# Nemesis1303/gFedNTM

Measured on AMD Instinct MI355X. Metric: docs/sec (whole node) + NPMI, ProdLDA K=50 8-client fed on synthetic BoW, higher is better.
Workload: dtype fp32

## Files before the change

### csrc/gfk_common.h

```cpp
#pragma once

#include <hip/hip_runtime.h>
#include <stdint.h>

#define GFK_MAX_LAYERS 8
#define GFK_MAX_SEGS 48
#define GFK_ADAM_CHUNK 256
#define GFK_WAVE 64

extern "C" {

enum GfkAct { GFK_SOFTPLUS = 0, GFK_RELU = 1, GFK_SIGMOID = 2, GFK_TANH = 3,
              GFK_LEAKYRELU = 4, GFK_ELU = 5, GFK_SELU = 6, GFK_RRELU = 7 };

enum GfkModelKind { GFK_PRODLDA = 0, GFK_LDA = 1 };

enum GfkInput { GFK_IN_BOW = 0, GFK_IN_COMBINED = 1, GFK_IN_CONTEXTUAL = 2 };

typedef struct GfkModel {
  int32_t bmax;
  int32_t V, K;
  int32_t n_hidden;
  int32_t H[GFK_MAX_LAYERS];
  int32_t act;
// ... 80 lines not shown
  int32_t ctx_kb, ctx_ckb;
  int32_t slot_cap;
  int32_t* ws_sidx;
  float* ws_sval;
  int32_t mm_bf16;
  int32_t ctx_parts;

  int32_t lab_on;
  int32_t lab_off;
  const float* labels;
  float *w_cls, *b_cls;
  float *ws_lab;
  float *ws_dlab;
  float *ws_ce;
  float *ws_thd;
  int32_t lab_in_enc;
  int32_t bwd_pre;
  float* ws_dt;
  const void* dev;
  const void* dev_upd;
  int32_t n_batch;
  int32_t ldb;
  int32_t ctx_bgrid;
  float* ws_colstat;
  float* kl_hist;
  float* rl_hist;
  int64_t off_own;
} GfkModel;

constexpr int GFK_FWD_POSTFOLD = 65536;
constexpr int GFK_LB = 524288;
constexpr int GFK_POST_ROWS2 = 1048576;
constexpr int GFK_POST_JOINT = 2097152;
constexpr int GFK_POST_ROWS4 = 4194304;
constexpr int GFK_BWD_BATCH8 = 8388608;
__host__ __device__ __forceinline__ int gfk_post_joint_rows(int stage_flags) {
  return !(stage_flags & GFK_POST_JOINT) ? 1 : (stage_flags & GFK_POST_ROWS4) ? 4 : 2;
}
constexpr int GFK_BMAX_LIMIT = 512;
__host__ __device__ __forceinline__ int gfk_hlast(const GfkModel& m) {
  int h = m.H[0];
#pragma unroll
  for (int l = 1; l < GFK_MAX_LAYERS; ++l) {
#if defined(__HIP_DEVICE_COMPILE__)
    const int hl = __builtin_amdgcn_readfirstlane(m.H[l]);
#else
    const int hl = m.H[l];
#endif
    if (l < m.n_hidden) h = hl;
  }
// ... 564 lines not shown
```

### csrc/posterior.hip

```cpp
#define GFK_BATCHED_COPY 1
#include "gfk_common.h"
#include "gfk_launch.h"

using namespace gfk;

namespace {
constexpr int PT = 256;
constexpr int FT = 1024;
__host__ __device__ inline int pad4(int x) { return (x + 3) & ~3; }

__device__ __forceinline__ float quad_sum(float v) {
  v += dpp_f<0xB1>(v);
  return v + dpp_f<0x4E>(v);
}

__host__ __device__ inline int post_hmax(const GfkModel& m) {
  int h = 0;
#pragma unroll
  for (int l = 0; l < GFK_MAX_LAYERS; ++l)
    if (l < m.n_hidden) h = h > m.H[l] ? h : m.H[l];
  return h;
}

__host__ __device__ inline int post_weight_floats(const GfkModel& m) {
// ... 361 lines not shown
  if (m.lab_on) post_label_head(m, red, row, nb, tid);
  GFK_STAMP(m, 3);
}

extern "C" size_t gfk_row_bwd_smem(const GfkModel* m) { return sizeof(float) * 4 * (size_t)pad4(m->K); }

__device__ __forceinline__ void post_term_hist(const GfkModel& m, int nb, int step0, float* scratch,
                                               int tid, int nt) {
  float k = 0.f, r = 0.f;
  for (int b = tid; b < nb; b += nt) {
    k += m.ws_kl[b];
    r += m.ws_rl[b];
  }
  lds_barrier();
  const float ks = block_sum_wave0(k, scratch);
  lds_barrier();
  const float rs = block_sum_wave0(r, scratch);
  if (tid == 0) {
    m.kl_hist[step0] = ks / (float)nb;
    m.rl_hist[step0] = rs / (float)nb;
  }
}

__device__ __forceinline__ void post_batch_level(const GfkModel& m, int nb, float* scratch, int tid) {
  __shared__ float red[3 * PT];
  const int K = m.K;
  const float wk = m.kl_weight;
  const int step0 = *m.step;
  float lterm = 0.f;
  for (int b = tid; b < nb; b += PT)
    lterm += wk * m.ws_kl[b] + m.ws_rl[b] + (m.lab_on ? m.ws_ce[b] : 0.f);
  if (m.learn_priors) {
    constexpr int RB = 16;
    const int cw = K <= 64 ? 64 : K <= 128 ? 128 : PT, ng = PT / cw;
    const int c = tid % cw, g = tid / cw;
    for (int k0 = 0; k0 < K; k0 += cw) {
      const int k = k0 + c, kk = min(k, K - 1);
      const float pm = m.prior_mean[kk];
      float smu = 0.f, svar = 0.f, sdm2 = 0.f;
      for (int r0 = g; r0 < nb; r0 += RB * ng) {
        float mu[RB], ls[RB];
#pragma unroll
        for (int i = 0; i < RB; ++i) {
          const int r = min(r0 + ng * i, nb - 1);
          mu[i] = m.ws_mu[r * K + kk];
          ls[i] = m.ws_ls[r * K + kk];
        }
#pragma unroll
        for (int i = 0; i < RB; ++i)
          if (r0 + ng * i < nb) {
            smu += mu[i];
            svar += expf(ls[i]);
            const float dm = pm - mu[i];
            sdm2 += dm * dm;
          }
      }
      red[tid] = smu;
      red[PT + tid] = svar;
      red[2 * PT + tid] = sdm2;
      lds_barrier();
      if (g == 0 && k < K) {
        for (int j = 1; j < ng; ++j) {
          smu += red[c + j * cw];
          svar += red[PT + c + j * cw];
          sdm2 += red[2 * PT + c + j * cw];
        }
        const float pv = m.prior_var[k];
        m.prior_mean[k + m.off_g] = wk * ((float)nb * pm - smu) / pv;
        m.prior_var[k + m.off_g] = wk * 0.5f * ((float)nb / pv - svar / (pv * pv) - sdm2 / (pv * pv));
      }
      lds_barrier();
    }
  }
  const float l = block_sum_wave0(lterm, scratch);
  if (tid == 0) {
    m.loss_hist[step0] = l;
    *m.step = step0 + 1;
  }
  if (m.kl_hist) post_term_hist(m, nb, step0, scratch, tid, PT);
}

template <int KQ, bool GB = false>
__global__ void __launch_bounds__(PT) gfk_row_bwd_k(GfkArgT<GB> ga) {
  const GfkModel& m = gfk_model(ga);
  extern __shared__ __attribute__((aligned(16))) float part[];
  int K = m.K, B = m.bmax, np = m.n_dpart + (m.lab_on ? 1 : 0);
  const float* dpart = m.ws_dthetad;
  const int32_t* nbp = m.ws_nb;
  keep(K, B, np, dpart, nbp);
  const int tid = threadIdx.x, lane = tid & 63, wave = uniform(tid >> 6);
  const int row = gfk_bx();
  const int nb = *nbp;
  if ((m.stage_flags & GFK_POST_ROWS2) && row == B) {
    post_batch_level(m, nb, part, tid);
    return;
  }
  if (row >= nb) return;
  GFK_STAMP(m, 8);
  constexpr int U = 32 / KQ;
// ... 288 lines not shown
  for (int q = 0; q < CQ; ++q) rs[q] = m.ws_bn_rstd[min(tid + q * FT, 2 * K - 1)];
  float lterm = 0.f, pmk = 0.f, pvk = 1.f;
  int step0 = 0;
  if (extra) {
    if (tid < nb) lterm = m.kl_weight * m.ws_kl[tid] + m.ws_rl[tid] + (m.lab_on ? m.ws_ce[tid] : 0.f);
    if (tid < K) { pmk = m.prior_mean[tid]; pvk = m.prior_var[tid]; }
    if (tid == 0) step0 = *m.step;
  }
  if (row >= nb && !extra) {
    vm_barrier();
    return;
  }
  vm_barrier();
  GFK_STAMP(m, 11);

  const float* dmu = in_lds ? smem + L.dmu : dmu_g;
  const float* dls = in_lds ? smem + L.dls : dls_g;
  const float* mu = in_lds ? smem + L.mu : mu_g;
  const float* ls = in_lds ? smem + L.ls : ls_g;
  float* S = smem + L.sums;
  const int P2 = pad4(2 * K);
  const float inv_nb = 1.f / (float)nb;
  if (extra) {
    const float* pmean = smem + L.pm;
    if constexpr (in_lds) {
      for (int cb = 0; cb < 2 * K; cb += FT / 16) {
        const int c2 = cb + (tid >> 4), g = tid & 15;
        const bool valid = c2 < 2 * K;
        const int k = c2 < K ? c2 : c2 - K;
        const float* xh = c2 < K ? mu : ls;
        const float pm = pmean[k];
        float s3 = 0.f, s4 = 0.f;
        if (valid)
#pragma unroll 4
          for (int r = g; r < nb; r += 16) {
            const float x = xh[r * LD + k];
            s3 += c2 < K ? x : expf(x);
            const float dm = pm - x;
            s4 += c2 < K ? dm * dm : 0.f;
          }
        s3 = row16_sum(s3);
        s4 = row16_sum(s4);
        if (valid && g == 0) {
          S[2 * P2 + c2] = s3;
          S[3 * P2 + c2] = s4;
        }
      }
    } else if constexpr (PS) {
      for (int c = tid; c < 2 * K; c += FT) {
        S[2 * P2 + c] = m.ws_colstat[8 * K + c];
        S[3 * P2 + c] = m.ws_colstat[10 * K + c];
      }
    } else {
      if (B <= 64) post_prior_sums<32>(K, nb, mu, ls, pmean, S + 2 * P2, S + 3 * P2, smem + L.red2, tid);
      else post_prior_sums<64>(K, nb, mu, ls, pmean, S + 2 * P2, S + 3 * P2, smem + L.red2, tid);
    }
    lds_barrier();
    const float wk = m.kl_weight;
    if (tid < K && m.learn_priors) {
      const float sdm2 = S[3 * P2 + tid];
      const float smu = S[2 * P2 + tid], svar = S[2 * P2 + K + tid];
      m.prior_mean[tid + m.off_g] = wk * ((float)nb * pmk - smu) / pvk;
      m.prior_var[tid + m.off_g] =
          wk * 0.5f * ((float)nb / pvk - svar / (pvk * pvk) - sdm2 / (pvk * pvk));
    }
    const float l = block_sum_wave0(lterm, smem + L.red);
    if (tid == 0) {
      m.loss_hist[step0] = l;
      *m.step = step0 + 1;
    }
    if (m.kl_hist) post_term_hist(m, nb, step0, smem + L.red, tid, FT);
    return;
  }
  if constexpr (in_lds) {
    for (int cb = 0; cb < 2 * K; cb += FT / 16) {
      const int c2 = cb + (tid >> 4), g = tid & 15;
      const bool valid = c2 < 2 * K;
      const int k = c2 < K ? c2 : c2 - K;
      const float* dy = c2 < K ? dmu : dls;
      const float* xh = c2 < K ? mu : ls;
      float s1 = 0.f, s2 = 0.f;
      if (valid)
#pragma unroll 4
        for (int r = g; r < nb; r += 16) {
          const float d = dy[r * LD + k], x = xh[r * LD + k];
          s1 += d;
          s2 += d * x;
        }
      s1 = row16_sum(s1);
      s2 = row16_sum(s2);
      if (valid && g == 0) {
// ... 398 lines not shown
```

### gfedntm_amd/data/bow.py

```python
from __future__ import annotations

import dataclasses
from typing import Dict, List, Optional, Sequence

import numpy as np
import scipy.sparse as sp
import torch
from torch.utils.data import Dataset


def to_csr(x) -> sp.csr_matrix:
    if isinstance(x, torch.Tensor):
        x = x.detach().cpu().numpy()
    m = sp.csr_matrix(x, dtype=np.float32)
    m.sum_duplicates()
    m.sort_indices()
    return m


class BOWDataset(Dataset):

    def __init__(self, X, idx2token):
        self.csr = to_csr(X)
        self.idx2token = idx2token
# ... 117 lines not shown
    def n_steps(self) -> int:
        return len(self.start)

    @staticmethod
    def build(n_docs: int, batch_size: int, n_steps: int, seed: int = 0) -> "BatchPlan":
        if n_docs <= 0:
            raise ValueError("empty shard")
        per_epoch = -(-n_docs // batch_size)
        n_epochs = -(-n_steps // per_epoch) if n_steps else 0
        rng = np.random.default_rng(seed)
        order = np.concatenate([rng.permutation(n_docs) for _ in range(max(n_epochs, 1))])
        s = np.arange(n_steps)
        ep, mb = s // per_epoch, s % per_epoch
        start = ep * n_docs + mb * batch_size
        size = np.minimum(batch_size, n_docs - mb * batch_size)
        return BatchPlan(order.astype(np.int32), start.astype(np.int32), size.astype(np.int32),
                         ep.astype(np.int32), mb.astype(np.int32), mb == per_epoch - 1,
                         n_docs, batch_size)

    def batch(self, step: int) -> np.ndarray:
        return self.order[self.start[step]: self.start[step] + self.size[step]]


def corpus_from_texts(texts: Sequence[str], vocabulary: Dict[str, int]) -> sp.csr_matrix:
    from .vocab import vectorize
    return vectorize(texts, vocabulary)


def stack_shards(shards: List[sp.csr_matrix]) -> sp.csr_matrix:
    return sp.vstack(shards, format="csr")
```

### gfedntm_amd/federation/client.py

```python
from __future__ import annotations

import datetime
import logging
from typing import List, Optional

import numpy as np
import torch

from ..data.bow import BatchPlan
from ..eval.export import postprocess_thetas, save_model_as_npz


class FederatedClient:
    def __init__(self, client_id: int, tm, dataset, max_iters: int, logger=None, seed: int = 0,
                 save_path: Optional[str] = None, log_every: int = 0, n_samples: int = 20,
                 epoch_snapshots: bool = False, agg: str = "params"):
        if agg not in ("params", "grads"):
            raise ValueError("agg must be 'params' (FedAvg) or 'grads' (gradient all-reduce)")
        self.agg = agg
        self.id = client_id
        self.tm = tm
        self.dataset = dataset
        self.logger = logger or logging.getLogger(f"gfedntm_amd.client{client_id}")
        self.save_path = save_path
        self.log_every = log_every
        self.n_samples = n_samples
        self.epoch_snapshots = epoch_snapshots
        tm.train_data = dataset
        self.data = tm.device_data(dataset)
        self.n_docs = self.data.n_docs
        self.max_iters = max_iters
        self.plan = BatchPlan.build(self.n_docs, tm.batch_size, max_iters, seed=seed)
        if agg == "grads" and tm.backend == "fused":
            from ..ops.engine import UPDATE_GRAD
            tm.engine.set_update_mode(UPDATE_GRAD)
        tm.engine.bind_data(self.data, self.plan)
        if hasattr(tm.engine, "own_rng"):
            tm.engine.own_rng(seed)
        tm.model.train()
        self.weight: Optional[float] = None
        self.ground_truth = None
        self.synthetic_eval: Optional[dict] = None
        self.current_mb = 0
        self.current_epoch = 0
        self.samples_processed = 0
        self.train_loss = 0.0
        self.epoch_first_step = 0
        self.results_saved = False
        tm.best_components = tm.model.beta
        self._pending: List[tuple] = []
        self._pinned = None
        self._events: List = []
        self._slot = 0
        hist = tm.engine.loss_hist
        if hist.device.type == "cuda":
            self._pinned = torch.zeros(64, dtype=torch.float32, pin_memory=True)
            self._events = [torch.cuda.Event() for _ in range(self._pinned.numel())]
            self._pinned[:1].copy_(hist[:1].sum().view(1), non_blocking=True)
            torch.cuda.synchronize(hist.device)

    @property
    def shared(self) -> torch.Tensor:
        return self.tm.flat.shared

    @property
    def fused(self) -> bool:
        return self.tm.backend == "fused"

    def set_fedavg_weight(self, w: float):
        self.weight = float(w)
        if self.fused and self.agg == "params":
            self.tm.engine.set_fedavg_scale(self.weight)

    def enable_graph(self, on: bool = True):
        if self.fused:
            self.tm.engine.enable_graph(on)

    def local_step(self, it: int):
        if self.agg == "grads":
            self.tm.engine.compute_grads(it)
            if self.weight is not None:
                self.shared_grads.mul_(self.weight)
            return
        self.tm.engine.step(it)
        if self.weight is not None and not self.fused:
# ... 34 lines not shown
                                 self.current_mb, loss, self.samples_processed,
                                 float(e.kl_hist[it].item()), float(e.rl_hist[it].item()))
            else:
                self.logger.info("-- -- Minibatch %d loss %s / samples processes %d", self.current_mb,
                                 loss, self.samples_processed)
        self.current_mb += 1
        if bool(self.plan.epoch_end[it]):
            self._queue_epoch_summary(self.epoch_first_step, it)
            if self.epoch_snapshots and self.save_path:
                self.flush()
                self.save_results(self.save_path.replace(".npz", f"_epoch_{self.current_epoch}.npz"))
            self.current_epoch += 1
            self.current_mb = 0
            self.epoch_first_step = it + 1
        if self.current_epoch >= self.tm.num_epochs and not self.results_saved:
            self.flush()
            self.logger.info("Epoch end reached")
            if self.save_path:
                self.save_results(self.save_path)
            self.results_saved = True
        self.poll()
        return self.results_saved

    def _queue_epoch_summary(self, first: int, last: int):
        hist = self.tm.engine.loss_hist
        if hist.device.type != "cuda":
            self._pending.append((self.current_epoch, self.samples_processed,
                                  float(hist[first: last + 1].sum()), None))
            self.poll()
            return
        if len(self._pending) >= self._pinned.numel():
            self.flush()
        slot = self._slot
        self._slot = (slot + 1) % self._pinned.numel()
        dst = self._pinned[slot: slot + 1]
        dst.copy_(hist[first: last + 1].sum().view(1), non_blocking=True)
        ev = self._events[slot]
        ev.record()
        self._pending.append((self.current_epoch, self.samples_processed, dst, ev))

    def _emit(self, epoch: int, samples: int, epoch_loss: float):
        self.train_loss += epoch_loss
        self.train_loss /= samples
        self.logger.info("Epoch: [%d/%d]\tSamples: [%d/%d]\tTrain Loss: %s\tTime: %s",
                         epoch + 1, self.tm.num_epochs, samples,
                         self.n_docs * self.tm.num_epochs, self.train_loss,
                         datetime.datetime.now())
# ... 71 lines not shown
```

### gfedntm_amd/federation/rank_round.py

```python
from __future__ import annotations

import os
from typing import Dict, List, Optional

import torch

from ..parallel.aggregator import (LOCAL_ALL, LOCAL_BCAST, LOCAL_FIRST, LOCAL_REFRESH,
                                   LOCAL_SHARED, LOCAL_SHARED_ALL, CollectiveAggregator,
                                   local_fedavg, prepare_local_fedavg)
from ..utils.misc import graph_capture
from .client import FederatedClient


def inplace_threshold_bytes() -> int:
    return int(float(os.environ.get("GFEDNTM_XGMI_INPLACE_MB", "8")) * (1 << 20))


class SingleClientRound:

    def __init__(self, client: FederatedClient, world: int, device, on_gpu_plane: bool,
                 allreduce: Optional[str], agg_mode: str, bucket_bytes: int, logger,
                 wire: str = "fp32"):
        self.clients = [client]
        self.client = client
        self.agg_mode = agg_mode
        if wire != "fp32" and agg_mode != "params":
            raise ValueError("fedavg_wire bf16delta averages parameters (agg_mode 'params')")
        self.wire = wire
        self.agg = CollectiveAggregator(bucket_bytes=bucket_bytes, method="rccl", wire=wire,
                                        weight=client.weight if wire != "fp32" else None)
        self.agg.set_reference(client.shared)
        self.in_step = None
        if on_gpu_plane and client.fused and agg_mode == "params" and world > 1:
            self.in_step = client.tm.engine.attach_fedavg(method=allreduce, wire=wire)
            logger.info("-- -- FedAvg all-reduce: %s", self.in_step)
        self.method = self.in_step if self.in_step else (None if world == 1 else "rccl")
        self.attach = getattr(client.tm.engine, "fedavg_attach", None) if self.in_step else None

    @property
    def xgmi(self) -> bool:
        return bool(self.in_step) and self.in_step.startswith("xgmi")

    def rounds_per_replay(self) -> int:
        c = self.client
        if not (c.fused and self.agg_mode == "params" and c.tm.engine.steps_per_replay_ok()
                and (self.in_step is not None or self.agg.world == 1)):
            return 1
        return max(1, int(os.environ.get("GFEDNTM_ROUNDS_PER_GRAPH", "16")))

    def prewarm(self, kmax: int):
        e = self.client.tm.engine
        if self.rounds_per_replay() <= 1 or e.plan is None:
            return
        e.warm_graph()
        k = 2
        while k <= kmax:
            if k not in e._graphs_k:
                e._capture(k)
            k *= 2

# ... 20 lines not shown
            self.agg.allreduce_(c.shared)

    def resync_reference(self):
        if self.wire == "fp32":
            return
        self.agg.set_reference(self.client.shared)
        if self.in_step is not None:
            self.client.tm.engine.fedavg_set_reference()

    def error(self) -> int:
        e = self.client.tm.engine
        return e.fedavg_error() if self.in_step is not None and self.client.fused else 0

    def error_async(self):
        self.client.tm.engine.fedavg_error_async()

    def error_poll(self) -> int:
        return self.client.tm.engine.fedavg_error_poll()

    def debug(self) -> dict:
        return self.client.tm.engine.fedavg_debug() if self.in_step is not None else {}

    def close(self):
        if self.in_step is not None and self.client.fused:
            self.client.tm.engine.detach_fedavg()
            self.in_step = None


class MultiClientRound:

    def __init__(self, clients: List[FederatedClient], world: int, device, on_gpu_plane: bool,
                 allreduce: Optional[str], graph: bool, logger, wire: str = "fp32"):
        self.clients = clients
        self.wire = wire
        self.weight = sum(c.weight for c in clients) if wire != "fp32" else None
        self.device = device
        self.world = world
        self.shared = [c.shared for c in clients]
        engines = [c.tm.engine for c in clients]
        self.fused = all(c.fused for c in clients) and device.type == "cuda"
        n = self.shared[0].numel()
        self.parts: Dict[str, tuple] = {"rest": (0, n)}
        from ..ops.engine import UPDATE_FUSED
        if (self.fused and world > 1 and on_gpu_plane
                and all(e.update_mode == UPDATE_FUSED for e in engines)):
            self.parts = dict(engines[0].fedavg_parts())
# ... 11 lines not shown
                           "inplace": {k: c.xgmi is not None and c.xgmi.data is not None
                                       for k, c in self.colls.items()},
                           "tuning": {k: c.tuning for k, c in self.colls.items() if c.tuning},
                           "plane": {k: c.describe() for k, c in self.colls.items()}}
        self.coll_in_graph = bool(self.colls) and all(c.xgmi is not None for c in self.colls.values())
        if not self.coll_in_graph and len(self.parts) > 1:
            for c in self.colls.values():
                if c.xgmi is not None:
                    c.xgmi.close()
                    c.xgmi = None
            self.parts = {"rest": (0, n)}
            coll = CollectiveAggregator(method="rccl", wire=wire, weight=self.weight)
            coll.prepare(self.shared[0])
            self.colls = {"rest": coll}
        self.method = (None if world == 1 else
                       "xgmi" + ("+overlap" if len(self.parts) > 1 else "")
                       if self.coll_in_graph else self.colls["rest"].active)
        self.graph = (graph and self.fused and not any(e.host_gemm_fallback for e in engines))
        if self.graph:
            for c in clients:
                c.enable_graph(False)
        if self.fused:
            prepare_local_fedavg(self.shared)
        self.fold_plan: Optional[str] = None
        self._g = None
        self._gk: Dict[int, object] = {}
        self._gm: Dict[int, object] = {}
        self._bss: Dict[tuple, object] = {}
        self._shared_plan: Optional[bool] = None
        self._shared_why: Optional[str] = None
        self._S: Optional[torch.Tensor] = None
        self._s_live = False
        self._gens = None
        self._streams = None
        self._side = None
        self._err = None
        if logger is not None:
            logger.info("-- -- FedAvg: %d local clients folded in-rank, %s across %d ranks",
                        len(clients), self.method or "no collective", world)

    def _states_equal(self) -> bool:
        s0 = self.shared[0]
        return all(torch.equal(s0, s) for s in self.shared[1:])

    def _fold(self, part: str, mode: int):
        a, b = self.parts[part]
        if len(self.shared) > 1 and b > a:
            local_fedavg(self.shared, mode, off=a, n=b - a)

    def _reduce_part(self, part: str):
        if not self.colls:
            self._fold(part, LOCAL_ALL)
            return
        self._fold(part, LOCAL_FIRST)
        a, b = self.parts[part]
        self.colls[part].allreduce_(self.shared[0][a:b])
        self._fold(part, LOCAL_BCAST)

    def _fork(self, part: str):
        main = torch.cuda.current_stream(self.device)
        side, ev_join, forks = self._side
        ev = forks[part]
# ... 238 lines not shown
        xs = self._xgmis()
        if not xs:
            return
        if self._err is None:
            self._err = {"host": torch.zeros(len(xs), dtype=torch.int32, pin_memory=True),
                         "ev": torch.cuda.Event(), "pending": False}
        for i, x in enumerate(xs):
            x.error_async(self._err["host"][i:i + 1])
        self._err["ev"].record()
        self._err["pending"] = True

    def error_poll(self) -> int:
        e = self._err
        if not e or not e["pending"] or not e["ev"].query():
            return 0
        e["pending"] = False
        return int(e["host"].max().item())

    def debug(self) -> dict:
        return {k: c.xgmi.debug_state() for k, c in self.colls.items() if c.xgmi is not None}

    def close(self):
        self._drop_graphs()
        for c in self.colls.values():
            if c.xgmi is not None:
                c.xgmi.close()
                c.xgmi = None
```

### gfedntm_amd/federation/runner.py

```python
from __future__ import annotations

import datetime
import logging
import os
import time
from typing import Dict, List, Optional, Sequence

import numpy as np
import torch

from ..data.bow import BOWDataset, CTMDataset
from ..data.vocab import union_vocabulary, vocabulary_dict
from ..eval.export import save_model_as_npz, server_model_path
from ..parallel.aggregator import CollectiveAggregator, LocalAggregator, fedavg_weights
from ..utils import checkpoint as ckpt
from ..utils.config import DEFAULT_GRADS_TO_SHARE, model_kwargs_from_params
from ..utils.logging import MetricsWriter
from ..utils.misc import graph_capture
from ..utils.trace import RoundWindow, trace_range
from .client import FederatedClient
from .data import ClientCorpus


CTM_TYPES = ("ctm", "zeroshot")


def shared_keys_for(model, grads_to_share: Sequence[str]) -> List[str]:
    want = set(grads_to_share)
    return [k for k in model.state_dict().keys() if k in want]


def make_topic_model(model_type: str, params: Dict, input_size: int, device,
                     backend: str = "auto", grads_to_share: Sequence[str] = DEFAULT_GRADS_TO_SHARE,
                     contextual_size: Optional[int] = None, seed: Optional[int] = None,
                     logger=None):
    from ..models import AVITM, CombinedTM, ZeroShotTM
    kw = model_kwargs_from_params(params)
    kw.setdefault("model_type", "prodLDA")
    kw["verbose"] = False
    if model_type == "avitm":
        cls = AVITM
    elif model_type in CTM_TYPES:
        cls = CombinedTM if model_type == "ctm" else ZeroShotTM
        kw["contextual_size"] = int(contextual_size or params.get("contextual_size", 768))
# ... 27 lines not shown
    return out


def record_terms(clients, on: bool):
    if on:
        for c in clients:
            c.tm.engine.record_terms(True)


def federation_coherence(tm, datas, topk: int = 10, matrix: str = "beta", per_topic: bool = False,
                         group=False, n_clients: Optional[int] = None) -> Dict:
    from ..eval.metrics import _federated_cooccurrence
    topics = tm.top_word_indices(topk, matrix)
    words = torch.unique(topics)
    counts, n_docs, engine = _federated_cooccurrence(datas, words, group)
    out = tm._coherence_result(topics, words, counts, n_docs, engine, topk, per_topic)
    out["clients"] = len(datas) if n_clients is None else int(n_clients)
    return out


def log_coherence(logger, coh: Dict, topk: int):
    logger.info("-- -- Global NPMI@%d: %.4f (TD %.4f, %d documents, %d clients)", topk,
                float(np.mean(coh["per_topic"])), coh["diversity"], coh["n_docs"], coh["clients"])


class LocalFederation:

    def __init__(self, corpora: Sequence[ClientCorpus], params: Dict, model_type: str = "avitm",
                 max_iters: int = 100, device=None, backend: str = "auto",
                 grads_to_share: Sequence[str] = DEFAULT_GRADS_TO_SHARE, seed: int = 0,
                 save_client: Optional[str] = None, save_server: Optional[str] = None,
                 logger=None, graph: bool = True, log_every: int = 0,
                 stop_at_num_epochs: bool = False, checkpoint_dir: Optional[str] = None,
                 checkpoint_every: int = 0, stamp: Optional[str] = None,
                 metrics_path: Optional[str] = None, metrics_every: int = 0, agg: str = "params",
                 round_graph: Optional[bool] = None, round_streams: bool = True,
                 groups: Optional[Sequence[int]] = None, round_batched: Optional[bool] = None,
                 fedavg_wire: str = "fp32"):
        self.logger = logger or logging.getLogger("gfedntm_amd.federation")
        self.agg_mode = agg
        if fedavg_wire != "fp32" and agg != "params":
            raise ValueError("fedavg_wire bf16delta averages parameters (agg 'params')")
        self.metrics = MetricsWriter(metrics_path)
        self.metrics_every = int(metrics_every)
        self.device = torch.device(device) if device is not None else \
            torch.device("cuda" if torch.cuda.is_available() else "cpu")
# ... 36 lines not shown
               and self.agg._native([c.shared for c in self.clients]))
        self.round_graph = can if round_graph is None else (bool(round_graph) and can)
        self.round_streams = bool(round_streams)
        self.round_batched = (round_batched if round_batched is not None else
                              os.environ.get("GFEDNTM_ROUND_BATCHED", "1") == "1")
        self._batched = None
        self.fold_plan: Optional[str] = None
        self._rg = None
        self._rgk = {}
        self._rg_gens = None
        self._stop = False
        if self.round_graph:
            for c in self.clients:
                c.enable_graph(False)
        self.round = 0
        if checkpoint_dir:
            starts = {ckpt.load_client_checkpoint(checkpoint_dir, c) for c in self.clients}
            if len(starts) != 1:
                raise RuntimeError(f"inconsistent client checkpoints: rounds {sorted(starts)}")
            self.round = starts.pop()
            if self.round:
                self.logger.info("-- -- Resuming the federation at round %d", self.round)
            self.agg.set_reference(self.clients[0].shared)

    def _sync(self):
        if self.device.type == "cuda":
            torch.cuda.synchronize(self.device)

    def _capture_round(self, k: int = 1):
        engines = [c.tm.engine for c in self.clients]
        for e in engines:
            e.prepare_external_capture()
        g = torch.cuda.CUDAGraph()
        shared = [c.shared for c in self.clients]
        self.agg.prepare(shared)
        self._batched = None
        if self.round_batched:
            from ..ops.engine import BatchedSteps
            sizes = self.agg.groups or [len(engines)]
            parts, o = [], 0
            for s in sizes:
                parts.append(engines[o:o + s])
                o += s
            if all(BatchedSteps.possible(p) for p in parts):
                self._batched_parts = [BatchedSteps(p) for p in parts]
                self._batched = self._batched_parts[0]
# ... 47 lines not shown
            c.tm.engine.sync_step_counter(it)
        if self._rg_gens != self._engine_gens():
            self._rg, self._rgk = None, {}
        if k not in self._rgk:
            self._capture_round(k)
        self._rgk[k][0].replay()
        for c in self.clients:
            c.tm.engine.advance_host_step(it + k - 1)

    def prewarm(self, kmax: int):
        if self._rg_gens != self._engine_gens():
            self._rg, self._rgk = None, {}
        k = 1
        while k <= kmax:
            if k not in self._rgk:
                self._capture_round(k)
            k *= 2

    def rounds_per_replay(self) -> int:
        if not self.round_graph:
            return 1
        return max(1, int(os.environ.get("GFEDNTM_ROUNDS_PER_GRAPH", "16")))

    def _run_end(self, it: int, kmax: int, ends, timed_end: int) -> int:
        r = it
        while r < it + kmax - 1 and r not in ends and r != timed_end:
            n1 = r + 1
            if ((self.metrics_every and n1 % self.metrics_every == 0)
                    or (self.checkpoint_dir and self.checkpoint_every
                        and n1 % self.checkpoint_every == 0)):
                break
            r += 1
        return r

    def _round(self, it: int, k: int = 1):
        if self.round_graph:
            self._round_graph_step(it, k)
            return
        for c in self.clients:
            c.local_step(it)
        if self.agg_mode == "grads":
            self.agg.average_([c.shared_grads for c in self.clients], prescaled=True)
            for c in self.clients:
                c.apply_step(it)
            packs = [c.pack_buffers() for c in self.clients]
            self.agg.average_(packs, prescaled=True)
            for c, p in zip(self.clients, packs):
                c.unpack_buffers(p)
        else:
            self.agg.average_([c.shared for c in self.clients], prescaled=True)

    def run(self, timing_warmup: int = 0) -> Dict:
        t0 = time.perf_counter()
        start = self.round
        timed_from = start
        last = start - 1
        self._stop = False
        win = RoundWindow(self._sync)
        ev = (torch.cuda.Event(enable_timing=True), torch.cuda.Event(enable_timing=True)) \
            if (self.device.type == "cuda" and timing_warmup) else None
        kmax = self.rounds_per_replay()
        ends = {self.max_iters - 1}
        if kmax > 1:
            self.prewarm(kmax)
            for c in self.clients:
                ends.update(int(i) for i in np.flatnonzero(c.plan.epoch_end))
                ends.update(int(i) for i in c.host_heavy_rounds())
        timed_end = start + timing_warmup - 1 if timing_warmup else -1
        covered = start - 1
        with trace_range("rounds"):
            for it in range(self.round, self.max_iters):
                if it > covered:
                    k = 1
                    if kmax > 1:
                        k = 1 << ((self._run_end(it, kmax, ends, timed_end) - it + 1).bit_length() - 1)
                    self._round(it, k)
                    covered = it + k - 1
                done = [c.end_round(it) for c in self.clients]
                self._after_round(it, win, done)
                last = it
                if timing_warmup and it == start + timing_warmup - 1:
                    self._sync()
                    t0 = time.perf_counter()
                    if ev is not None:
                        ev[0].record()
                    timed_from = it + 1
                    win.reset()
                if self._stop:
                    break
        if ev is not None:
            ev[1].record()
        self._sync()
        wall = time.perf_counter() - t0
        device_s = ev[0].elapsed_time(ev[1]) * 1e-3 if ev is not None and timed_from > start else None
        n_rounds = last + 1 - timed_from
        docs = sum(int(c.plan.size[timed_from:last + 1].sum()) for c in self.clients) \
            if n_rounds > 0 else 0
        for c in self.clients:
# ... 265 lines not shown

    def meet(where: str):
        sync()
        check_comm(where)
        dist.barrier(group=ctrl)

    dist.barrier(group=ctrl)
    if probe is not None:
        sync()
        digest_now(start - 1)
    debug_comm = os.environ.get("GFEDNTM_COMM_DEBUG") == "1" and rr.xgmi
    t_dbg0 = time.perf_counter()
    win = RoundWindow(sync)
    ev = (torch.cuda.Event(enable_timing=True), torch.cuda.Event(enable_timing=True)) \
        if (device.type == "cuda" and timing_warmup) else None
    t0 = time.perf_counter()
    timed_from = start
    last = start - 1
    kmax = getattr(rr, "rounds_per_replay", lambda: 1)()
    if round_hook is not None or corrupt_from is not None or debug_comm:
        kmax = 1
    ends = set(align) | {stop_after}
    if kmax > 1:
        for c in clients:
            ends.update(int(i) for i in np.flatnonzero(c.plan.epoch_end))
        if timing_warmup:
            ends.add(start + timing_warmup - 1)

    def host_after(r: int) -> bool:
        n1 = r + 1
        return bool(r in ends
                    or (poll_every and n1 % poll_every == 0) or (digest_every and n1 % digest_every == 0)
                    or (metrics_every and n1 % metrics_every == 0)
                    or (checkpoint_dir and checkpoint_every and n1 % checkpoint_every == 0))

    def run_end(it: int) -> int:
        r = it
        while r < it + kmax - 1 and not host_after(r):
            r += 1
        return r

    if kmax > 1 and hasattr(rr, "prewarm"):
        rr.prewarm(kmax)
    covered = start - 1
    with trace_range("rounds"):
        for it in range(start, stop_after + 1):
            if hb is not None:
                hb.mark(it, 0)
            if it > covered:
                k = 1 << ((run_end(it) - it + 1).bit_length() - 1) if kmax > 1 else 1
                more = kmax > 1 and not host_after(it + k - 1)
                if k > 1:
                    rr.step(it, hb, k, more=more)
                else:
                    rr.step(it, hb, more=more)
                covered = it + k - 1
            elif hb is not None:
                hb.mark(it, 1)
            if corrupt_from is not None and it >= corrupt_from:
                _flip_word(clients[0].shared)
            if debug_comm and it < start + 16:
                t_dbg = time.perf_counter()
                sync()
                logger.warning("rank %d round %d: enqueued at %.3f s, done at %.3f s, xGMI "
                               "error %d", rank, it, t_dbg - t_dbg0, time.perf_counter() - t_dbg0,
                               rr.error())
            heavy = it in align
            if heavy:
                sync()
                check_comm(f"the host work of round {it}")
                digest_now(it)
                if hb is not None:
                    hb.busy(True)
            for c in clients:
# ... 65 lines not shown
```

### gfedntm_amd/ops/engine.py

```python
from __future__ import annotations

import ctypes as C
import os
from typing import Dict, List, Optional, Tuple

import numpy as np
import torch
import torch.nn.functional as F

from ..data.bow import BatchPlan, DeviceCSR
from ..models.engine import EngineBase
from ..utils.flat import ALIGN, slot_view
from ..utils.misc import graph_capture
from . import kernel_abi as abi
from . import native

BMAX_CHOICES = (16, 32, 64, 128, 256, 512)
LB_MIN_BMAX = 256
LDS_LIMIT = 160 * 1024
CTX_INFER_ROWS = 256
VB = 64
STAGE_PLANS = (1, 0, 3, 2)
STAGE_FWD_STRIP = 4
STAGE_WIN_SPARSE = 16
STAGE_CTX_FULL = 32
STAGE_WIN_BATCH8 = 512
STAGE_CTX_BWDPP = 4096
STAGE_CTX_RS = 32768
STAGE_FWD_POSTFOLD = 65536
STAGE_LB = 524288
STAGE_POST_ROWS2 = abi.POST_ROWS2
STAGE_POST_JOINT = abi.POST_JOINT
STAGE_POST_ROWS4 = abi.POST_ROWS4
# ... 748 lines not shown
        m.ctx = data.contextual.data_ptr() if data.contextual is not None else None
        if m.stage_flags & STAGE_CTX_RS and data.contextual is not None \
                and 4 * data.contextual.numel() >= (1 << 31):
            m.stage_flags &= ~STAGE_CTX_RS
            m.ctx_parts = 0
        if m.lab_on:
            if data.labels is None or data.labels.shape[1] != m.L:
                raise ValueError(f"the model has a label head of size {m.L}: bind data with "
                                 f"labels [n_docs, {m.L}]")
            m.labels = data.labels.data_ptr()
        cap = max(16, -(-int(data.row_len_max) // 16) * 16)
        if self.ws.get("sidx") is None or self.ws["sidx"].numel() < self.bmax * cap:
            self.ws["sidx"] = torch.zeros(self.bmax * cap + 16, dtype=torch.int32, device=dev)
            self.ws["sval"] = torch.zeros(self.bmax * cap + 16, dtype=torch.float32, device=dev)
        m.slot_cap = cap
        m.ws_sidx, m.ws_sval = self.ws["sidx"].data_ptr(), self.ws["sval"].data_ptr()
        m.plan_order = self._plan_dev["order"].data_ptr()
        m.plan_start = self._plan_dev["start"].data_ptr()
        m.plan_size = self._plan_dev["size"].data_ptr()
        m.loss_hist = self.loss_hist.data_ptr()
        m.kl_hist = self.kl_hist.data_ptr() if self.terms_on else None
        m.rl_hist = self.rl_hist.data_ptr() if self.terms_on else None
        m.n_steps = plan.n_steps
        self.d_step.zero_()
        self._host_step = 0
        self._invalidate_graph()
        self._launch([abi.PH_BATCH_PREP])

    def record_terms(self, on: bool = True):
        super().record_terms(on)
        if self.kl_hist is not None:
            self._m.kl_hist = self.kl_hist.data_ptr() if self.terms_on else None
            self._m.rl_hist = self.rl_hist.data_ptr() if self.terms_on else None
            self._invalidate_graph()

    def phases(self) -> List[int]:
        if self._m.kind == abi.KIND_LDA:
            ph = [p for p in abi.LDA_STEP if p != abi.PH_ADAM] + \
                ([abi.PH_ADAM] if self.update_mode == UPDATE_GRAD else [])
        else:
            ph = abi.PRODLDA_STEP + ([abi.PH_ADAM] if self.update_mode == UPDATE_GRAD else [])
            if self.large_batch:
                if not self._m.lb_fused & 1:
                    ph.insert(ph.index(abi.PH_PRODLDA_FWD), abi.PH_LB_GEMM_FWD)
                if not self._m.lb_fused & 2:
                    ph.insert(ph.index(abi.PH_PRODLDA_BWD) + 1, abi.PH_LB_GEMM_BWD)
            if self._m.stage_flags & STAGE_FWD_POSTFOLD:
                ph.remove(abi.PH_POST_FWD)
        if self.ctx_fused:
            if self._m.ctx_fused == 1:
                ph.insert(ph.index(abi.PH_ENC_FWD), abi.PH_CTXF_FWD)
                ph.insert(ph.index(abi.PH_ENC_BWD), abi.PH_CTXF_BWD)
        elif self.kind == "ctm":
            ph.insert(ph.index(abi.PH_ENC_FWD), abi.PH_CTX_FWD)
            ph.insert(ph.index(abi.PH_ENC_BWD) + 1, abi.PH_CTX_BWD)
        if self._comm is not None and self._comm["mode"] == "graph":
            if "beta" in self._comm:
# ... 399 lines not shown
        self.d_step.copy_(saved[0])
        self.adam_t.copy_(saved[1])
        self.adam_pow.copy_(saved[2])
        self.adam_coef.copy_(saved[3])
        if k == 1:
            self._graph = g
        else:
            self._graphs_k[k] = g

    def warm_graph(self):
        if self.graph_enabled and self._graph is None:
            self._capture()

    def prepare_external_capture(self):
        self._sync_dev()
        if self.host_gemm_fallback:
            self._warm_host_gemms()

    def launch_step_phases(self):
        if self._comm is not None:
            raise RuntimeError("external capture is for in-process federations (no collective)")
        self._launch(self.phases())

    def advance_host_step(self, s: int):
        self._host_step = s + 1

    def sync_step_counter(self, s: int):
        if s != self._host_step:
            self.d_step.fill_(s)
            self._host_step = s
            self._launch([abi.PH_BATCH_PREP])

    @property
    def grad_buffer(self) -> torch.Tensor:
        return self.grad

    def compute_grads(self, s: int) -> torch.Tensor:
        if self.update_mode != UPDATE_GRAD or self.fedavg_scale is not None:
            raise RuntimeError("gradient aggregation needs gradient mode without the FedAvg pre-scale")
        if self.plan is None:
            raise RuntimeError("bind_data() first")
        self.sync_step_counter(s)
        self._launch([p for p in self.phases() if p not in (abi.PH_ADAM, abi.PH_FEDAVG_BETA,
                                                           abi.PH_FEDAVG_WA, abi.PH_FEDAVG_END)])
        self._host_step = s + 1
        return self.loss_hist[s]

    def apply_grads(self, s: int):
        self._launch([abi.PH_ADAM])

    def step(self, s: int) -> torch.Tensor:
        if self.plan is None:
# ... 288 lines not shown
```

### gfedntm_amd/ops/kernel_abi.py

```python
from __future__ import annotations

import ctypes as C

MAX_LAYERS = 8
MAX_SEGS = 48
P = C.c_void_p

ACT_CODES = {"softplus": 0, "relu": 1, "sigmoid": 2, "tanh": 3, "leakyrelu": 4, "elu": 5,
             "selu": 6, "rrelu": 7}
KIND_PRODLDA, KIND_LDA = 0, 1
IN_BOW, IN_COMBINED, IN_CONTEXTUAL = 0, 1, 2

POST_ROWS2 = 1 << 20
POST_JOINT = 1 << 21
POST_ROWS4 = 1 << 22
POST_ROWS_SHAPES = {"serial2": POST_ROWS2, "2": POST_ROWS2 | POST_JOINT,
                    "4": POST_ROWS2 | POST_JOINT | POST_ROWS4}

BWD_BATCH8 = 1 << 23

PH_BATCH_DOCS = 0
PH_ENC_FWD = 1
PH_POST_FWD = 2
PH_PRODLDA_FWD = 3
# ... 51 lines not shown
        ("step", P), ("adam_t", P), ("loss_hist", P),
        ("ws_doc", P), ("ws_nb", P), ("ws_z", P * MAX_LAYERS), ("ws_a", P * MAX_LAYERS), ("ws_hd", P), ("ws_mask_h", P),
        ("ws_mu_raw", P), ("ws_ls_raw", P), ("ws_mu", P), ("ws_ls", P), ("ws_bn_rstd", P),
        ("ws_eps", P), ("ws_theta", P), ("ws_mask_t", P), ("ws_thetad", P),
        ("ws_kl", P), ("ws_rl", P), ("ws_lse", P), ("ws_s", P),
        ("ws_zn", P), ("ws_col_rstd", P), ("ws_row_part", P), ("ws_dthetad", P),
        ("ws_dz", P * MAX_LAYERS), ("ws_dmr", P), ("ws_dlr", P),
        ("ws_dmu", P), ("ws_dls", P),
        ("ws_dbsm", P), ("ws_ck", P), ("ws_hctx", P), ("ws_tstart", P), ("ws_erange", P),
        ("ws_next", P), ("dbg", P),
        ("lr", C.c_float), ("beta1", C.c_float), ("beta2", C.c_float), ("adam_eps", C.c_float),
        ("weight_decay", C.c_float), ("fed_scale", C.c_float), ("update_mode", C.c_int32),
        ("fed_scale_on", C.c_int32), ("flat_base", P), ("n_shared", C.c_int64),
        ("off_m", C.c_int64), ("off_v", C.c_int64), ("off_g", C.c_int64),
        ("adam_pow", P), ("adam_coef", P), ("ws_dtheta", P),
        ("w_a", P), ("b_a", P), ("ws_actx", P), ("ws_hpart", P),
        ("ctx_fused", C.c_int32), ("ctx_kb", C.c_int32), ("ctx_ckb", C.c_int32),
        ("slot_cap", C.c_int32), ("ws_sidx", P), ("ws_sval", P),
        ("mm_bf16", C.c_int32), ("ctx_parts", C.c_int32),
        ("lab_on", C.c_int32), ("lab_off", C.c_int32), ("labels", P), ("w_cls", P), ("b_cls", P),
        ("ws_lab", P), ("ws_dlab", P), ("ws_ce", P), ("ws_thd", P),
        ("lab_in_enc", C.c_int32), ("bwd_pre", C.c_int32), ("ws_dt", P),
        ("dev", P), ("dev_upd", P), ("n_batch", C.c_int32), ("ldb", C.c_int32),
        ("ctx_bgrid", C.c_int32), ("ws_colstat", P),
        ("kl_hist", P), ("rl_hist", P),
        ("off_own", C.c_int64),
    ]


class GfkWJob(C.Structure):
    _fields_ = [("param", P), ("dz", P), ("a", P), ("rows", C.c_int32), ("cols", C.c_int32),
                ("j0", C.c_int32), ("i0", C.c_int32)]


class GfkVJob(C.Structure):
    _fields_ = [("param", P), ("src", P), ("n", C.c_int32), ("pad", C.c_int32)]


MAX_WJOBS, MAX_VJOBS = 40, 16


class GfkUpdate(C.Structure):
    _fields_ = [("n_w", C.c_int32), ("n_v", C.c_int32), ("w", GfkWJob * MAX_WJOBS),
                ("v", GfkVJob * MAX_VJOBS)]


ADAM_CHUNK = 256
SOLVER_CODES = {"adam": 0, "sgd": 1, "adagrad": 2, "adadelta": 3, "rmsprop": 4}

# ... 145 lines not shown
```

Baseline: 4.699 million.

## Accumulate per-epoch loss sums on device so multi-round graphs span epoch ends

The posterior kernels now keep a running per-epoch loss sum on the device and write it into a shared slots tensor indexed by epoch. A ring of pinned buffers and events lets clients fetch epoch summaries asynchronously. Because summaries no longer need a host sync, epoch ends are dropped from the round-cut set, so longer multi-round graphs can run without breaking at each epoch boundary. It also adds a lazy materialise hook for shared client state, and it depends on the running-sum seeding being correct after a step counter resync.

Result: faster. 4.919 million (median of 6 runs) (+4.7%).

```diff
diff --git a/csrc/gfk_common.h b/csrc/gfk_common.h
--- a/csrc/gfk_common.h
+++ b/csrc/gfk_common.h
@@ -126,10 +126,14 @@
   int32_t n_batch;
   int32_t ldb;
   int32_t ctx_bgrid;
+  int32_t epoch_stride;
   float* ws_colstat;
   float* kl_hist;
   float* rl_hist;
   int64_t off_own;
+  const int32_t* epoch_idx;
+  float* epoch_run;
+  float* epoch_loss;
 } GfkModel;
 
 constexpr int GFK_FWD_POSTFOLD = 65536;
diff --git a/csrc/posterior.hip b/csrc/posterior.hip
--- a/csrc/posterior.hip
+++ b/csrc/posterior.hip
@@ -407,14 +407,30 @@
   }
 }
 
+__device__ __forceinline__ void post_epoch_sum(const GfkModel& m, int step0, int ecur, int eprev,
+                                               float run, float l) {
+  asm volatile("" : "+v"(ecur), "+v"(eprev), "+v"(run));
+  const float cum = (step0 == 0 || eprev != ecur) ? l : run + l;
+  *m.epoch_run = cum;
+  m.epoch_loss[(int64_t)ecur * m.epoch_stride] = cum;
+}
+
 __device__ __forceinline__ void post_batch_level(const GfkModel& m, int nb, float* scratch, int tid) {
   __shared__ float red[3 * PT];
   const int K = m.K;
   const float wk = m.kl_weight;
   const int step0 = *m.step;
+  const bool esum = m.epoch_loss != nullptr;
+  float erun = 0.f;
+  int ecur = 0, eprev = 0;
+  if (esum && tid == 0) erun = *m.epoch_run;
   float lterm = 0.f;
   for (int b = tid; b < nb; b += PT)
     lterm += wk * m.ws_kl[b] + m.ws_rl[b] + (m.lab_on ? m.ws_ce[b] : 0.f);
+  if (esum && tid == 0) {
+    ecur = m.epoch_idx[step0];
+    eprev = m.epoch_idx[max(step0 - 1, 0)];
+  }
   if (m.learn_priors) {
     constexpr int RB = 16;
     const int cw = K <= 64 ? 64 : K <= 128 ? 128 : PT, ng = PT / cw;
@@ -460,6 +476,7 @@
   const float l = block_sum_wave0(lterm, scratch);
   if (tid == 0) {
     m.loss_hist[step0] = l;
+    if (esum) post_epoch_sum(m, step0, ecur, eprev, erun, l);
     *m.step = step0 + 1;
   }
   if (m.kl_hist) post_term_hist(m, nb, step0, scratch, tid, PT);
@@ -794,6 +811,14 @@
   const int P2 = pad4(2 * K);
   const float inv_nb = 1.f / (float)nb;
   if (extra) {
+    const bool esum = m.epoch_loss != nullptr;
+    float erun = 0.f;
+    int ecur = 0, eprev = 0;
+    if (esum && tid == 0) {
+      erun = *m.epoch_run;
+      ecur = m.epoch_idx[step0];
+      eprev = m.epoch_idx[max(step0 - 1, 0)];
+    }
     const float* pmean = smem + L.pm;
     if constexpr (in_lds) {
       for (int cb = 0; cb < 2 * K; cb += FT / 16) {
@@ -839,6 +864,7 @@
     const float l = block_sum_wave0(lterm, smem + L.red);
     if (tid == 0) {
       m.loss_hist[step0] = l;
+      if (esum) post_epoch_sum(m, step0, ecur, eprev, erun, l);
       *m.step = step0 + 1;
     }
     if (m.kl_hist) post_term_hist(m, nb, step0, smem + L.red, tid, FT);
diff --git a/gfedntm_amd/data/bow.py b/gfedntm_amd/data/bow.py
--- a/gfedntm_amd/data/bow.py
+++ b/gfedntm_amd/data/bow.py
@@ -163,6 +163,14 @@
         return self.order[self.start[step]: self.start[step] + self.size[step]]
 
 
+def epoch_index(epoch_end: np.ndarray) -> np.ndarray:
+    end = np.asarray(epoch_end, dtype=bool)
+    out = np.zeros(len(end), dtype=np.int32)
+    if len(end) > 1:
+        out[1:] = np.cumsum(end[:-1], dtype=np.int64)
+    return out
+
+
 def corpus_from_texts(texts: Sequence[str], vocabulary: Dict[str, int]) -> sp.csr_matrix:
     from .vocab import vectorize
     return vectorize(texts, vocabulary)
diff --git a/gfedntm_amd/federation/client.py b/gfedntm_amd/federation/client.py
--- a/gfedntm_amd/federation/client.py
+++ b/gfedntm_amd/federation/client.py
@@ -7,11 +7,13 @@
 import numpy as np
 import torch
 
-from ..data.bow import BatchPlan
+from ..data.bow import BatchPlan, epoch_index
 from ..eval.export import postprocess_thetas, save_model_as_npz
 
 
 class FederatedClient:
+    _shared_hook = None
+
     def __init__(self, client_id: int, tm, dataset, max_iters: int, logger=None, seed: int = 0,
                  save_path: Optional[str] = None, log_every: int = 0, n_samples: int = 20,
                  epoch_snapshots: bool = False, agg: str = "params"):
@@ -52,6 +54,9 @@
         self._pinned = None
         self._events: List = []
         self._slot = 0
+        self._esums = None
+        self._ecol = 0
+        self._epoch_of = epoch_index(self.plan.epoch_end)
         hist = tm.engine.loss_hist
         if hist.device.type == "cuda":
             self._pinned = torch.zeros(64, dtype=torch.float32, pin_memory=True)
@@ -61,6 +66,8 @@
 
     @property
     def shared(self) -> torch.Tensor:
+        if self._shared_hook is not None:
+            self._shared_hook()
         return self.tm.flat.shared
 
     @property
@@ -141,7 +148,14 @@
         self.poll()
         return self.results_saved
 
+    def attach_epoch_sums(self, reader, col: int):
+        self._esums, self._ecol = reader, int(col)
+
     def _queue_epoch_summary(self, first: int, last: int):
+        if self._esums is not None:
+            dst, ev = self._esums.fetch(last, int(self._epoch_of[last]), self._ecol)
+            self._pending.append((self.current_epoch, self.samples_processed, dst, ev))
+            return
         hist = self.tm.engine.loss_hist
         if hist.device.type != "cuda":
             self._pending.append((self.current_epoch, self.samples_processed,
diff --git a/gfedntm_amd/federation/epoch_sums.py b/gfedntm_amd/federation/epoch_sums.py
--- /dev/null
+++ b/gfedntm_amd/federation/epoch_sums.py
@@ -0,0 +1,79 @@
+from __future__ import annotations
+
+import os
+from typing import Dict, List, Optional, Tuple
+
+import torch
+
+RING = 64
+
+
+def epoch_sums_mode() -> str:
+    mode = os.environ.get("GFEDNTM_EPOCH_SUMS", "device")
+    if mode not in ("device", "host"):
+        raise ValueError("GFEDNTM_EPOCH_SUMS must be 'device' or 'host'")
+    return mode
+
+
+class EpochSums:
+
+    def __init__(self, clients: List):
+        self.clients = list(clients)
+        engines = [c.tm.engine for c in self.clients]
+        dev = engines[0].device
+        M = len(engines)
+        n_epochs = max(int(e.n_epochs) for e in engines)
+        self.slots = torch.zeros(max(n_epochs, 1), M, dtype=torch.float32, device=dev)
+        self._pinned = torch.zeros(RING, M, dtype=torch.float32, pin_memory=True)
+        self._events = [torch.cuda.Event() for _ in range(RING)]
+        self._next = 0
+        self._round: Optional[int] = None
+        self._by_epoch: Dict[int, int] = {}
+        for i, (c, e) in enumerate(zip(self.clients, engines)):
+            e.bind_epoch_sums(self.slots, i)
+            c.attach_epoch_sums(self, i)
+        self.enqueue(0, 0)
+        torch.cuda.synchronize(dev)
+
+    @staticmethod
+    def attach(clients: List) -> Optional["EpochSums"]:
+        ok = epoch_sums_mode() == "device" and bool(clients)
+        for c in clients:
+            e = c.tm.engine
+            ok = ok and (getattr(c, "fused", False) and hasattr(e, "bind_epoch_sums")
+                         and e.device.type == "cuda" and e.plan is not None)
+        if not ok:
+            EpochSums.detach(clients)
+            return None
+        return EpochSums(clients)
+
+    @staticmethod
+    def detach(clients: List):
+        for c in clients:
+            if c._esums is not None:
+                c.attach_epoch_sums(None, 0)
+            e = c.tm.engine
+            if getattr(e, "epoch_sums", None) is not None:
+                e.bind_epoch_sums(None)
+
+    def enqueue(self, epoch: int, slot: int):
+        self._pinned[slot].copy_(self.slots[epoch], non_blocking=True)
+        self._events[slot].record()
+
+    def _reclaim(self, slot: int):
+        ev = self._events[slot]
+        for c in self.clients:
+            if any(p[3] is ev for p in c._pending):
+                c.flush()
+
+    def fetch(self, it: int, epoch: int, col: int) -> Tuple[torch.Tensor, torch.cuda.Event]:
+        if it != self._round:
+            self._round, self._by_epoch = it, {}
+        slot = self._by_epoch.get(epoch)
+        if slot is None:
+            slot = self._next
+            self._next = (slot + 1) % RING
+            self._reclaim(slot)
+            self.enqueue(epoch, slot)
+            self._by_epoch[epoch] = slot
+        return self._pinned[slot, col:col + 1], self._events[slot]
diff --git a/gfedntm_amd/federation/rank_round.py b/gfedntm_amd/federation/rank_round.py
--- a/gfedntm_amd/federation/rank_round.py
+++ b/gfedntm_amd/federation/rank_round.py
@@ -10,6 +10,7 @@
                                    local_fedavg, prepare_local_fedavg)
 from ..utils.misc import graph_capture
 from .client import FederatedClient
+from .epoch_sums import EpochSums
 
 
 def inplace_threshold_bytes() -> int:
@@ -36,6 +37,7 @@
             logger.info("-- -- FedAvg all-reduce: %s", self.in_step)
         self.method = self.in_step if self.in_step else (None if world == 1 else "rccl")
         self.attach = getattr(client.tm.engine, "fedavg_attach", None) if self.in_step else None
+        self.epoch_sums = EpochSums.attach(self.clients)
 
     @property
     def xgmi(self) -> bool:
@@ -102,6 +104,8 @@
         return self.client.tm.engine.fedavg_debug() if self.in_step is not None else {}
 
     def close(self):
+        EpochSums.detach(self.clients)
+        self.epoch_sums = None
         if self.in_step is not None and self.client.fused:
             self.client.tm.engine.detach_fedavg()
             self.in_step = None
@@ -159,6 +163,7 @@
                 c.enable_graph(False)
         if self.fused:
             prepare_local_fedavg(self.shared)
+        self.epoch_sums = EpochSums.attach(clients)
         self.fold_plan: Optional[str] = None
         self._g = None
         self._gk: Dict[int, object] = {}
@@ -172,9 +177,19 @@
         self._streams = None
         self._side = None
         self._err = None
+        for c in clients:
+            c._shared_hook = self._materialise
         if logger is not None:
             logger.info("-- -- FedAvg: %d local clients folded in-rank, %s across %d ranks",
                         len(clients), self.method or "no collective", world)
+
+    def _materialise(self):
+        if self._s_live:
+            if torch.cuda.is_current_stream_capturing():
+                raise RuntimeError("a client's shared state was asked for inside a graph capture")
+            for s in self.shared:
+                s.copy_(self._S)
+            self._s_live = False
 
     def _states_equal(self) -> bool:
         s0 = self.shared[0]
@@ -459,6 +474,11 @@
 
     def close(self):
         self._drop_graphs()
+        self._materialise()
+        for c in self.clients:
+            c._shared_hook = None
+        EpochSums.detach(self.clients)
+        self.epoch_sums = None
         for c in self.colls.values():
             if c.xgmi is not None:
                 c.xgmi.close()
diff --git a/gfedntm_amd/federation/runner.py b/gfedntm_amd/federation/runner.py
--- a/gfedntm_amd/federation/runner.py
+++ b/gfedntm_amd/federation/runner.py
@@ -20,6 +20,7 @@
 from ..utils.trace import RoundWindow, trace_range
 from .client import FederatedClient
 from .data import ClientCorpus
+from .epoch_sums import EpochSums
 
 
 CTM_TYPES = ("ctm", "zeroshot")
@@ -93,6 +94,40 @@
 def log_coherence(logger, coh: Dict, topk: int):
     logger.info("-- -- Global NPMI@%d: %.4f (TD %.4f, %d documents, %d clients)", topk,
                 float(np.mean(coh["per_topic"])), coh["diversity"], coh["n_docs"], coh["clients"])
+
+
+def round_cuts(epoch_ends, heavy, last: int, warmup_end: Optional[int] = None,
+               device_sums: bool = False) -> set:
+    ends = {int(r) for r in heavy} | {int(last)}
+    if warmup_end is not None:
+        ends.add(int(warmup_end))
+    if not device_sums:
+        ends.update(int(r) for r in epoch_ends)
+    return ends
+
+
+def host_after_round(r: int, ends, poll_every: int = 0, digest_every: int = 0,
+                     metrics_every: int = 0, checkpoint_every: int = 0) -> bool:
+    n1 = r + 1
+    return bool(r in ends
+                or (poll_every and n1 % poll_every == 0)
+                or (digest_every and n1 % digest_every == 0)
+                or (metrics_every and n1 % metrics_every == 0)
+                or (checkpoint_every and n1 % checkpoint_every == 0))
+
+
+def run_plan(it: int, kmax: int, ends, **every) -> tuple:
+    if kmax <= 1:
+        return 1, False
+    r = it
+    while r < it + kmax - 1 and not host_after_round(r, ends, **every):
+        r += 1
+    k = 1 << ((r - it + 1).bit_length() - 1)
+    return k, not host_after_round(it + k - 1, ends, **every)
+
+
+def client_epoch_ends(clients) -> List[int]:
+    return sorted({int(i) for c in clients for i in np.flatnonzero(c.plan.epoch_end)})
 
 
 class LocalFederation:
@@ -175,6 +210,7 @@
             if self.round:
                 self.logger.info("-- -- Resuming the federation at round %d", self.round)
             self.agg.set_reference(self.clients[0].shared)
+        self.epoch_sums = EpochSums.attach(self.clients)
 
     def _sync(self):
         if self.device.type == "cuda":
@@ -268,17 +304,6 @@
             return 1
         return max(1, int(os.environ.get("GFEDNTM_ROUNDS_PER_GRAPH", "16")))
 
-    def _run_end(self, it: int, kmax: int, ends, timed_end: int) -> int:
-        r = it
-        while r < it + kmax - 1 and r not in ends and r != timed_end:
-            n1 = r + 1
-            if ((self.metrics_every and n1 % self.metrics_every == 0)
-                    or (self.checkpoint_dir and self.checkpoint_every
-                        and n1 % self.checkpoint_every == 0)):
-                break
-            r += 1
-        return r
-
     def _round(self, it: int, k: int = 1):
         if self.round_graph:
             self._round_graph_step(it, k)
@@ -309,17 +334,17 @@
         ends = {self.max_iters - 1}
         if kmax > 1:
             self.prewarm(kmax)
-            for c in self.clients:
-                ends.update(int(i) for i in np.flatnonzero(c.plan.epoch_end))
-                ends.update(int(i) for i in c.host_heavy_rounds())
-        timed_end = start + timing_warmup - 1 if timing_warmup else -1
+            ends = round_cuts(client_epoch_ends(self.clients),
+                              [r for c in self.clients for r in c.host_heavy_rounds()],
+                              self.max_iters - 1, start + timing_warmup - 1 if timing_warmup else None,
+                              device_sums=self.epoch_sums is not None)
+        every = dict(metrics_every=self.metrics_every,
+                     checkpoint_every=self.checkpoint_every if self.checkpoint_dir else 0)
         covered = start - 1
         with trace_range("rounds"):
             for it in range(self.round, self.max_iters):
                 if it > covered:
-                    k = 1
-                    if kmax > 1:
-                        k = 1 << ((self._run_end(it, kmax, ends, timed_end) - it + 1).bit_length() - 1)
+                    k, _ = run_plan(it, kmax, ends, **every)
                     self._round(it, k)
                     covered = it + k - 1
                 done = [c.end_round(it) for c in self.clients]
@@ -631,23 +656,11 @@
         kmax = 1
     ends = set(align) | {stop_after}
     if kmax > 1:
-        for c in clients:
-            ends.update(int(i) for i in np.flatnonzero(c.plan.epoch_end))
-        if timing_warmup:
-            ends.add(start + timing_warmup - 1)
-
-    def host_after(r: int) -> bool:
-        n1 = r + 1
-        return bool(r in ends
-                    or (poll_every and n1 % poll_every == 0) or (digest_every and n1 % digest_every == 0)
-                    or (metrics_every and n1 % metrics_every == 0)
-                    or (checkpoint_dir and checkpoint_every and n1 % checkpoint_every == 0))
-
-    def run_end(it: int) -> int:
-        r = it
-        while r < it + kmax - 1 and not host_after(r):
-            r += 1
-        return r
+        ends = round_cuts(client_epoch_ends(clients), align, stop_after,
+                          start + timing_warmup - 1 if timing_warmup else None,
+                          device_sums=getattr(rr, "epoch_sums", None) is not None)
+    every = dict(poll_every=poll_every, digest_every=digest_every, metrics_every=metrics_every,
+                 checkpoint_every=checkpoint_every if checkpoint_dir else 0)
 
     if kmax > 1 and hasattr(rr, "prewarm"):
         rr.prewarm(kmax)
@@ -657,8 +670,7 @@
             if hb is not None:
                 hb.mark(it, 0)
             if it > covered:
-                k = 1 << ((run_end(it) - it + 1).bit_length() - 1) if kmax > 1 else 1
-                more = kmax > 1 and not host_after(it + k - 1)
+                k, more = run_plan(it, kmax, ends, **every)
                 if k > 1:
                     rr.step(it, hb, k, more=more)
                 else:
diff --git a/gfedntm_amd/ops/engine.py b/gfedntm_amd/ops/engine.py
--- a/gfedntm_amd/ops/engine.py
+++ b/gfedntm_amd/ops/engine.py
@@ -8,7 +8,7 @@
 import torch
 import torch.nn.functional as F
 
-from ..data.bow import BatchPlan, DeviceCSR
+from ..data.bow import BatchPlan, DeviceCSR, epoch_index
 from ..models.engine import EngineBase
 from ..utils.flat import ALIGN, slot_view
 from ..utils.misc import graph_capture
@@ -803,6 +803,14 @@
         m.kl_hist = self.kl_hist.data_ptr() if self.terms_on else None
         m.rl_hist = self.rl_hist.data_ptr() if self.terms_on else None
         m.n_steps = plan.n_steps
+        eidx = epoch_index(plan.epoch_end)
+        self.n_epochs = int(eidx[-1]) + 1 if len(eidx) else 0
+        self._epoch_of = eidx
+        self._plan_dev["epoch"] = torch.from_numpy(eidx).to(dev)
+        self.epoch_run = torch.zeros(1, dtype=torch.float32, device=dev)
+        self.epoch_sums = None
+        m.epoch_idx, m.epoch_run = None, None
+        m.epoch_loss, m.epoch_stride = None, 0
         self.d_step.zero_()
         self._host_step = 0
         self._invalidate_graph()
@@ -814,6 +822,28 @@
             self._m.kl_hist = self.kl_hist.data_ptr() if self.terms_on else None
             self._m.rl_hist = self.rl_hist.data_ptr() if self.terms_on else None
             self._invalidate_graph()
+
+    def bind_epoch_sums(self, slots: Optional[torch.Tensor], col: int = 0):
+        if self.plan is None:
+            raise RuntimeError("bind_data() first")
+        if torch.cuda.is_current_stream_capturing():
+            raise RuntimeError("bind_epoch_sums inside a graph capture")
+        m = self._m
+        if slots is None:
+            m.epoch_idx, m.epoch_run, m.epoch_loss, m.epoch_stride = None, None, None, 0
+        else:
+            if (slots.dtype != torch.float32 or slots.device != self.device or slots.dim() != 2
+                    or slots.shape[0] < self.n_epochs or not 0 <= col < slots.shape[1]
+                    or slots.stride(1) != 1):
+                raise ValueError("epoch sums: float32 [n_epochs or more, M] on the engine's "
+                                 "device, unit column stride, 0 <= col < M")
+            m.epoch_idx = self._plan_dev["epoch"].data_ptr()
+            m.epoch_run = self.epoch_run.data_ptr()
+            m.epoch_loss = slots.data_ptr() + 4 * int(col)
+            m.epoch_stride = int(slots.stride(0))
+            self.epoch_run.zero_()
+        self.epoch_sums = None if slots is None else slots[:, col]
+        self._invalidate_graph()
 
     def phases(self) -> List[int]:
         if self._m.kind == abi.KIND_LDA:
@@ -1259,12 +1289,27 @@
             raise RuntimeError("external capture is for in-process federations (no collective)")
         self._launch(self.phases())
 
+    def _seed_epoch_run(self, s: int):
+        self.epoch_run.zero_()
+        if self.epoch_sums is None or not 0 < s < len(self._epoch_of):
+            return
+        first = s
+        while first > 0 and self._epoch_of[first - 1] == self._epoch_of[s]:
+            first -= 1
+        if first < s:
+            hist = self.loss_hist[first:s].cpu().numpy()
+            acc = np.float32(hist[0])
+            for v in hist[1:]:
+                acc = np.float32(acc + v)
+            self.epoch_run.fill_(float(acc))
+
     def advance_host_step(self, s: int):
         self._host_step = s + 1
 
     def sync_step_counter(self, s: int):
         if s != self._host_step:
             self.d_step.fill_(s)
+            self._seed_epoch_run(s)
             self._host_step = s
             self._launch([abi.PH_BATCH_PREP])
 
diff --git a/gfedntm_amd/ops/kernel_abi.py b/gfedntm_amd/ops/kernel_abi.py
--- a/gfedntm_amd/ops/kernel_abi.py
+++ b/gfedntm_amd/ops/kernel_abi.py
@@ -97,9 +97,10 @@
         ("ws_lab", P), ("ws_dlab", P), ("ws_ce", P), ("ws_thd", P),
         ("lab_in_enc", C.c_int32), ("bwd_pre", C.c_int32), ("ws_dt", P),
         ("dev", P), ("dev_upd", P), ("n_batch", C.c_int32), ("ldb", C.c_int32),
-        ("ctx_bgrid", C.c_int32), ("ws_colstat", P),
+        ("ctx_bgrid", C.c_int32), ("epoch_stride", C.c_int32), ("ws_colstat", P),
         ("kl_hist", P), ("rl_hist", P),
         ("off_own", C.c_int64),
+        ("epoch_idx", P), ("epoch_run", P), ("epoch_loss", P),
     ]
 
 
```
